# VivianDLi/CryoVIT

Measured on NVIDIA B200. Metric: DINOv2 ViT-g/14 feature slices/sec, higher is better.
Workload: dtype fp16 (norm1 out, attention out, qkv/proj weights) + bf16 (q/k/v, probabilities, norm2 out, w12, FFN hidden, w3) operands, fp32 accumulate

## Files before the change

### cryovit_b200/csrc/attention_tcgen05.cu

```cuda
#include "ptx.cuh"
#include "tmap.h"

namespace cvit {

constexpr int FA_BQ = 128, FA_BK = 128, FA_D = 64;
constexpr int FA_THREADS = 512;
constexpr int FA_REGS_SOFTMAX = 184, FA_REGS_EPILOGUE = 72, FA_REGS_CONTROL = 72;
constexpr int FA_STAGES = 4;
constexpr int FA_TILE_BYTES = 128 * 128;
constexpr int FA_SMEM = (4 + 2 * FA_STAGES) * FA_TILE_BYTES + 4096  + 512  + 1024;
constexpr int FA_TMEM_COLS = 512;
constexpr uint32_t FA_COL_S = 0, FA_COL_P = 256, FA_COL_O = 384;

#ifdef CVIT_FA_TRACE
__device__ __forceinline__ unsigned long long fa_globaltimer() {
  unsigned long long t;
  asm volatile("mov.u64 %0, %%globaltimer;" : "=l"(t));
  return t;
}
#define FA_PROF_DECL uint32_t prof_acc[8] = {0, 0, 0, 0, 0, 0, 0, 0}; const unsigned long long prof_t0 = fa_globaltimer(); uint32_t prof_last = clock()
#define FA_PROF(slot) do { const uint32_t now_ = clock(); prof_acc[slot] += now_ - prof_last; prof_last = now_; } while (0)
#define FA_PROF_DUMP(tiles) do { if (args.trace && blockIdx.x < 4 && lane == 0) {                      \
    long long* d_ = args.trace + (blockIdx.x * 16 + warp) * 10;                                        \
    for (int i_ = 0; i_ < 8; ++i_) d_[i_] = prof_acc[i_];                                              \
    d_[8] = (tiles); d_[9] = (long long)(fa_globaltimer() - prof_t0); } } while (0)
#else
#define FA_PROF_DECL do { } while (0)
#define FA_PROF(slot) do { } while (0)
#define FA_PROF_DUMP(tiles) do { } while (0)
#endif
struct FaArgs {
  long long* trace;
  __nv_bfloat16* out;
  int T, heads, C, slices;
  float scale_log2e;
};

__device__ __forceinline__ uint64_t pack_f32x2(float lo, float hi) {
  uint64_t r;
  asm("mov.b64 %0, {%1, %2};" : "=l"(r) : "f"(lo), "f"(hi));
  return r;
}
__device__ __forceinline__ void unpack_f32x2(uint64_t v, float& lo, float& hi) {
  asm("mov.b64 {%0, %1}, %2;" : "=f"(lo), "=f"(hi) : "l"(v));
}
__device__ __forceinline__ uint64_t fma_f32x2(uint64_t a, uint64_t b, uint64_t c) {
  uint64_t r;
  asm("fma.rn.f32x2 %0, %1, %2, %3;" : "=l"(r) : "l"(a), "l"(b), "l"(c));
  return r;
}
__device__ __forceinline__ uint64_t add_f32x2(uint64_t a, uint64_t b) {
  uint64_t r;
  asm("add.rn.f32x2 %0, %1, %2;" : "=l"(r) : "l"(a), "l"(b));
  return r;
}
__device__ __forceinline__ float fmax3(float a, float b, float c) {
  float r;
  asm("max.f32 %0, %1, %2, %3;" : "=f"(r) : "f"(a), "f"(b), "f"(c));
  return r;
}

template <bool F16, bool OUT16, bool OUT32 = false>
__global__ void __launch_bounds__(FA_THREADS, 1)
attention_tcgen05_kernel(const __grid_constant__ CUtensorMap tmQKV, const FaArgs args) {
  extern __shared__ uint8_t smem_raw[];
  const uint32_t smem_base = (smem_u32(smem_raw) + 1023u) & ~1023u;
  const uint32_t sQ = smem_base;
  const uint32_t sK = smem_base + 4 * FA_TILE_BYTES;
  const uint32_t sV = smem_base + (4 + FA_STAGES) * FA_TILE_BYTES;
  const uint32_t sL = smem_base + (4 + 2 * FA_STAGES) * FA_TILE_BYTES;
  const uint32_t sBar = sL + 4096;
  const uint32_t bar_q = sBar, bar_q_empty = sBar + 16;
  const uint32_t bar_kv_full = sBar + 32;
  const uint32_t bar_kv_empty = sBar + 32 + 8 * FA_STAGES;
  const uint32_t bar_grp = sBar + 32 + 16 * FA_STAGES;
  constexpr uint32_t B_S = 0, B_SFREE = 8, B_P = 16, B_PV = 24, B_OFULL = 32, B_OEMPTY = 40, B_LFULL = 48;
  const uint32_t tmem_slot = bar_grp + 128;
  uint8_t* smem_gen = smem_raw + (smem_base - smem_u32(smem_raw));

  const int warp = threadIdx.x >> 5, lane = threadIdx.x & 31;
  const int T = args.T;
  const int n_tiles = (T + FA_BK - 1) / FA_BK;
  const int n_qt = (T + FA_BQ - 1) / FA_BQ;
  const int n_pairs = (n_qt + 1) >> 1;
  const int total_items = n_pairs * args.heads * args.slices;
  const bool ragged = (T % FA_BK) != 0;
  auto kv_tile = [&](int j) { return ragged ? (j == 0 ? n_tiles - 1 : j - 1) : j; };
  enum { PAIRED = 0, SPLIT = 1, SOLO = 2 };
  auto pair_kind = [&](int pair) { return 2 * pair + 1 < n_qt ? PAIRED : n_tiles > 1 ? SPLIT : SOLO; };
  auto item_kind = [&](int item) { return pair_kind(item % n_pairs); };
  auto mine = [&](int kind, int g, int j) { return kind == PAIRED || (kind == SPLIT ? (j & 1) == g : g == 0); };

  constexpr float FA_RESCALE_LOG2 = F16 ? 8.0f : 16.0f;
  if (threadIdx.x == 0) {
    tma_prefetch_desc(&tmQKV);
    for (int b = 0; b < 2; ++b) {
      mbar_init(bar_q + 8 * b, 1);
      mbar_init(bar_q_empty + 8 * b, 2);
    }
    for (int s = 0; s < FA_STAGES; ++s) {
      mbar_init(bar_kv_full + 8 * s, 1);
      mbar_init(bar_kv_empty + 8 * s, 2);
    }
    for (int g = 0; g < 2; ++g) {
      mbar_init(bar_grp + 64 * g + B_S, 1);
      mbar_init(bar_grp + 64 * g + B_SFREE, 4);
      mbar_init(bar_grp + 64 * g + B_P, 4);
      mbar_init(bar_grp + 64 * g + B_PV, 1);
      mbar_init(bar_grp + 64 * g + B_OFULL, 1);
      mbar_init(bar_grp + 64 * g + B_OEMPTY, 4);
      mbar_init(bar_grp + 64 * g + B_LFULL, 4);
    }
    fence_mbar_init();
  }
  if (warp == 13) tmem_alloc<FA_TMEM_COLS>(tmem_slot);
  tcgen05_fence_before();
  __syncthreads();
  tcgen05_fence_after();
  const uint32_t tmem_base = *reinterpret_cast<volatile uint32_t*>(smem_gen + (tmem_slot - smem_base));

  if (warp >= 12) {
    asm volatile("setmaxnreg.dec.sync.aligned.u32 %0;" ::"n"(FA_REGS_CONTROL));
    if (warp == 12) {
      if (lane == 0) {
        uint32_t kv_it = 0, k = 0;
        for (int item = blockIdx.x; item < total_items; item += gridDim.x, ++k) {
          const int pair = item % n_pairs, bh = item / n_pairs;
          const int head = bh % args.heads, slice = bh / args.heads;
          const int cq = head * FA_D, ck = args.C + head * FA_D, cv = 2 * args.C + head * FA_D;
          const uint32_t qb_ = k & 1, sQk = sQ + qb_ * 2 * FA_TILE_BYTES, bq = bar_q + 8 * qb_;
          mbar_wait(bar_q_empty + 8 * qb_, ((k >> 1) & 1) ^ 1u);
          mbar_arrive_expect_tx(bq, 2 * FA_TILE_BYTES);
          tma_load_3d(sQk, &tmQKV, bq, cq, (2 * pair) * FA_BQ, slice);
          const int qb = item_kind(item) == PAIRED ? 2 * pair + 1 : 2 * pair;
          tma_load_3d(sQk + FA_TILE_BYTES, &tmQKV, bq, cq, qb * FA_BQ, slice);
          for (int j = 0; j < n_tiles; ++j, ++kv_it) {
            const uint32_t s = kv_it % FA_STAGES;
            mbar_wait(bar_kv_empty + 8 * s, ((kv_it / FA_STAGES) & 1) ^ 1u);
            mbar_arrive_expect_tx(bar_kv_full + 8 * s, 2 * FA_TILE_BYTES);
            tma_load_3d(sK + s * FA_TILE_BYTES, &tmQKV, bar_kv_full + 8 * s, ck, kv_tile(j) * FA_BK, slice);
            tma_load_3d(sV + s * FA_TILE_BYTES, &tmQKV, bar_kv_full + 8 * s, cv, kv_tile(j) * FA_BK, slice);
          }
        }
      }
    } else if (warp <= 14) {
      const int g = warp - 13;
      const uint32_t bg = bar_grp + 64 * g;
      constexpr uint32_t idesc_pv = (F16 ? umma_idesc_f16_f32(FA_BQ, FA_D) : umma_idesc_bf16_f32(FA_BQ, FA_D)) | (1u << 16);
      auto n_mma_of = [&](int j) {
        const int valid = min(FA_BK, T - kv_tile(j) * FA_BK);
        return (valid + 15) & ~15;
      };
      FA_PROF_DECL;
      auto issue_s = [&](uint32_t tg, int j, uint32_t k, int commits_q) {
        const uint32_t kv = k * n_tiles + j;
        FA_PROF(7);
        if (tg > 0) mbar_wait(bg + B_SFREE, (tg - 1) & 1);
        FA_PROF(0);
        const uint32_t s = kv % FA_STAGES;
        mbar_wait(bar_kv_full + 8 * s, (kv / FA_STAGES) & 1);
        tcgen05_fence_after();
        FA_PROF(1);
        if (elect_one_sync()) {
          const uint32_t idesc_s = F16 ? umma_idesc_f16_f32(FA_BQ, n_mma_of(j)) : umma_idesc_bf16_f32(FA_BQ, n_mma_of(j));
          const uint64_t qd = umma_smem_desc_kmajor<128>(sQ + ((k & 1) * 2 + g) * FA_TILE_BYTES);
          const uint64_t kd = umma_smem_desc_kmajor<128>(sK + s * FA_TILE_BYTES);
          const uint32_t tS = tmem_base + FA_COL_S + g * 128;
#pragma unroll
          for (int kk = 0; kk < FA_D / 16; ++kk) umma_bf16(tS, qd + 2 * kk, kd + 2 * kk, idesc_s, kk > 0);
          for (int i = 0; i < commits_q; ++i) umma_commit(bar_q_empty + 8 * (k & 1));
          umma_commit(bg + B_S);
        }
        __syncwarp();
        FA_PROF(2);
      };
      auto issue_pv = [&](uint32_t tg, int j, uint32_t kv, bool first, bool last, uint32_t kg, int commits_kv) {
        FA_PROF(7);
        mbar_wait(bg + B_P, tg & 1);
        FA_PROF(3);
        if (first) mbar_wait(bg + B_OEMPTY, (kg & 1) ^ 1u);
        tcgen05_fence_after();
        FA_PROF(4);
        const uint32_t s = kv % FA_STAGES;
        if (elect_one_sync()) {
          const uint32_t tP = tmem_base + FA_COL_P + g * 64, tO = tmem_base + FA_COL_O + g * 64;
          const uint64_t vd = umma_smem_desc_mnmajor_sw128(sV + s * FA_TILE_BYTES, FA_TILE_BYTES);
          if (n_mma_of(j) == FA_BK) {
#pragma unroll
            for (int kk = 0; kk < FA_BK / 16; ++kk)
              umma_bf16_ts(tO, tP + 8 * kk, vd + 128 * kk, idesc_pv, !first || kk != 0);
          } else {
            for (int kk = 0; kk < n_mma_of(j) / 16; ++kk)
              umma_bf16_ts(tO, tP + 8 * kk, vd + 128 * kk, idesc_pv, !first || kk != 0);
          }
          for (int i = 0; i < commits_kv; ++i) umma_commit(bar_kv_empty + 8 * s);
          umma_commit(bg + B_PV);
          if (last) umma_commit(bg + B_OFULL);
        }
        __syncwarp();
        FA_PROF(5);
      };
      struct Cur { int item; uint32_t k; int pair; int kind; int j; };
      const int pair_step = gridDim.x % n_pairs;
      auto cur_valid = [&](const Cur& c) { return c.item < total_items; };
      auto first_j = [&](int kind) { return kind == SPLIT ? g : 0; };
      auto last_j = [&](int kind) { return kind == SPLIT ? n_tiles - 1 - ((n_tiles - 1 - g) & 1) : n_tiles - 1; };
      auto advance = [&](Cur& c) {
        for (;;) {
          ++c.j;
          if (c.j >= n_tiles) {
            c.item += gridDim.x;
            ++c.k;
            c.j = 0;
            if (c.item >= total_items) return;
            c.pair += pair_step;
            if (c.pair >= n_pairs) c.pair -= n_pairs;
            c.kind = pair_kind(c.pair);
          }
          if (mine(c.kind, g, c.j)) return;
        }
      };
      Cur cs{(int)blockIdx.x, 0u, (int)(blockIdx.x % n_pairs), 0, -1}, cp = cs;
      if (cur_valid(cs)) {
        cs.kind = cp.kind = pair_kind(cs.pair);
        advance(cs);
        advance(cp);
      }
      uint32_t ok = 0, obs_q = ~0u;
      int oj = 0;
      auto observe_up_to = [&](const Cur& c) {
        while (ok < c.k || (ok == c.k && oj < c.j)) {
          if (oj == 0) { mbar_wait(bar_q + 8 * (ok & 1), (ok >> 1) & 1); obs_q = ok; }
          const uint32_t kv = ok * n_tiles + oj;
          mbar_wait(bar_kv_full + 8 * (kv % FA_STAGES), (kv / FA_STAGES) & 1);
          if (++oj == n_tiles) { oj = 0; ++ok; }
        }
        if (oj == 0) { mbar_wait(bar_q + 8 * (ok & 1), (ok >> 1) & 1); obs_q = ok; }
        if (++oj == n_tiles) { oj = 0; ++ok; }
      };
      uint32_t ts = 0, tp = 0, kg = 0;
      auto do_s = [&]() {
        FA_PROF(7);
        observe_up_to(cs);
        FA_PROF(6);
        const bool last = cs.j == last_j(cs.kind);
        issue_s(ts, cs.j, cs.k, last ? (cs.kind == SOLO ? 2 : 1) : 0);
        ++ts;
        advance(cs);
      };
      if (cur_valid(cs)) do_s();
      while (cur_valid(cp)) {
        bool s_first = false;
        if (cur_valid(cs)) {
          if (cs.k == obs_q) s_first = true;
          else if (cs.k == obs_q + 1) s_first = __all_sync(0xffffffffu, mbar_try_wait(bar_q + 8 * (cs.k & 1), (cs.k >> 1) & 1));
        }
        if (s_first) do_s();
        const bool first = cp.j == first_j(cp.kind), last = cp.j == last_j(cp.kind);
        issue_pv(tp, cp.j, cp.k * n_tiles + cp.j, first, last, kg, cp.kind == PAIRED ? 1 : 2);
        ++tp;
        if (last) ++kg;
        advance(cp);
        if (!s_first && cur_valid(cs)) do_s();
      }
      FA_PROF(7);
      FA_PROF_DUMP(tp);
    }
  } else if (warp >= 8) {
    asm volatile("setmaxnreg.dec.sync.aligned.u32 %0;" ::"n"(FA_REGS_EPILOGUE));
    const int q = warp & 3;
    const int row = q * 32 + lane;
    const uint32_t t_row = tmem_base + (static_cast<uint32_t>(q * 32) << 16);
    const float* sL_gen = reinterpret_cast<const float*>(smem_gen + (sL - smem_base));
    const float c = args.scale_log2e;
    uint32_t kg[2] = {0, 0};
    for (int item = blockIdx.x; item < total_items; item += gridDim.x) {
      const int pair = item % n_pairs, bh = item / n_pairs, kind = item_kind(item);
      __nv_bfloat16* out_bh = args.out + ((size_t)(bh / args.heads) * T) * args.C + (bh % args.heads) * FA_D;
      float* outf_bh = reinterpret_cast<float*>(args.out) + ((size_t)(bh / args.heads) * T) * args.C + (bh % args.heads) * FA_D;
      if (kind == SPLIT) {
        const int qt = 2 * pair;
        const uint32_t pa = kg[0] & 1, pb = kg[1] & 1;
        ++kg[0];
        ++kg[1];
        mbar_wait(bar_grp + B_LFULL, pa);
        mbar_wait(bar_grp + 64 + B_LFULL, pb);
        const float la = sL_gen[(pa * 2 + 0) * 256 + row], ma = sL_gen[(pa * 2 + 0) * 256 + 128 + row];
        const float lb = sL_gen[(pb * 2 + 1) * 256 + row], mb = sL_gen[(pb * 2 + 1) * 256 + 128 + row];
        const float mm = fmaxf(ma, mb);
        float wa = ex2_approx((ma - mm) * c), wb = ex2_approx((mb - mm) * c);
        const float inv = 1.0f / (wa * la + wb * lb);
        wa *= inv;
        wb *= inv;
        mbar_wait(bar_grp + B_OFULL, pa);
        mbar_wait(bar_grp + 64 + B_OFULL, pb);
        tcgen05_fence_after();
        const bool warp_active = qt * FA_BQ + q * 32 < T;
        if (OUT32 && warp_active) {
          const int tok = qt * FA_BQ + row;
          uint4* dst = reinterpret_cast<uint4*>(outf_bh + (size_t)tok * args.C);
#pragma unroll 1
          for (int hh = 0; hh < 4; ++hh) {
            uint32_t oa[16], o2[16];
            tmem_ld_32x16(t_row + FA_COL_O + hh * 16, oa);
            tmem_ld_32x16(t_row + FA_COL_O + 64 + hh * 16, o2);
            tmem_ld_wait();
#pragma unroll
            for (int i = 0; i < 16; ++i)
              oa[i] = __float_as_uint(round_tf32(__uint_as_float(oa[i]) * wa + __uint_as_float(o2[i]) * wb));
            if (tok < T) {
#pragma unroll
              for (int i = 0; i < 4; ++i) dst[4 * hh + i] = make_uint4(oa[4 * i], oa[4 * i + 1], oa[4 * i + 2], oa[4 * i + 3]);
            }
          }
        } else if (warp_active) {
          const int tok = qt * FA_BQ + row;
          uint4* dst = reinterpret_cast<uint4*>(out_bh + (size_t)tok * args.C);
#pragma unroll 1
          for (int hh = 0; hh < 4; ++hh) {
            uint32_t oa[16], o2[16], ob[8];
            tmem_ld_32x16(t_row + FA_COL_O + hh * 16, oa);
            tmem_ld_32x16(t_row + FA_COL_O + 64 + hh * 16, o2);
            tmem_ld_wait();
#pragma unroll
            for (int i = 0; i < 8; ++i)
              ob[i] = pack_16x2<OUT16>(__uint_as_float(oa[2 * i]) * wa + __uint_as_float(o2[2 * i]) * wb,
                                  __uint_as_float(oa[2 * i + 1]) * wa + __uint_as_float(o2[2 * i + 1]) * wb);
            if (tok < T) {
              dst[2 * hh] = make_uint4(ob[0], ob[1], ob[2], ob[3]);
              dst[2 * hh + 1] = make_uint4(ob[4], ob[5], ob[6], ob[7]);
            }
          }
        }
        tcgen05_fence_before();
        __syncwarp();
        if (lane == 0) {
          mbar_arrive(bar_grp + B_OEMPTY);
          mbar_arrive(bar_grp + 64 + B_OEMPTY);
        }
        continue;
      }
#pragma unroll
      for (int g = 0; g < 2; ++g) {
        if (kind == SOLO && g == 1) continue;
        const int qt = 2 * pair + g;
        const uint32_t bg = bar_grp + 64 * g;
        const uint32_t par = kg[g] & 1;
        ++kg[g];
        mbar_wait(bg + B_LFULL, par);
        const float l = sL_gen[(par * 2 + g) * 256 + row];
        mbar_wait(bg + B_OFULL, par);
        tcgen05_fence_after();
        const bool warp_active = qt * FA_BQ + q * 32 < T;
        if (OUT32 && warp_active) {
          const float inv = 1.0f / l;
          const int tok = qt * FA_BQ + row;
          uint4* dst = reinterpret_cast<uint4*>(outf_bh + (size_t)tok * args.C);
#pragma unroll 1
          for (int hh = 0; hh < 4; ++hh) {
            uint32_t o[16];
            tmem_ld_32x16(t_row + FA_COL_O + g * 64 + hh * 16, o);
            tmem_ld_wait();
#pragma unroll
            for (int i = 0; i < 16; ++i) o[i] = __float_as_uint(round_tf32(__uint_as_float(o[i]) * inv));
            if (tok < T) {
#pragma unroll
              for (int i = 0; i < 4; ++i) dst[4 * hh + i] = make_uint4(o[4 * i], o[4 * i + 1], o[4 * i + 2], o[4 * i + 3]);
            }
          }
        } else if (warp_active) {
          const float inv = 1.0f / l;
          const int tok = qt * FA_BQ + row;
          uint4* dst = reinterpret_cast<uint4*>(out_bh + (size_t)tok * args.C);
#pragma unroll 1
          for (int hh = 0; hh < 2; ++hh) {
            uint32_t o[32];
            tmem_ld_32x32(t_row + FA_COL_O + g * 64 + hh * 32, o);
            tmem_ld_wait();
#pragma unroll
            for (int i = 0; i < 16; ++i) o[i] = pack_16x2<OUT16>(__uint_as_float(o[2 * i]) * inv, __uint_as_float(o[2 * i + 1]) * inv);
            if (tok < T) {
#pragma unroll
              for (int i = 0; i < 4; ++i) dst[4 * hh + i] = make_uint4(o[4 * i], o[4 * i + 1], o[4 * i + 2], o[4 * i + 3]);
            }
          }
        }
        tcgen05_fence_before();
        __syncwarp();
        if (lane == 0) mbar_arrive(bg + B_OEMPTY);
      }
    }
  } else {
    asm volatile("setmaxnreg.inc.sync.aligned.u32 %0;" ::"n"(FA_REGS_SOFTMAX));
    const int g = warp >> 2;
    const int q = warp & 3;
    const int row = q * 32 + lane;
    const uint32_t t_row = tmem_base + (static_cast<uint32_t>(q * 32) << 16);
    const uint32_t tS = t_row + FA_COL_S + g * 128, tP = t_row + FA_COL_P + g * 64, tO = t_row + FA_COL_O + g * 64;
    const uint32_t bg = bar_grp + 64 * g;
    const float c = args.scale_log2e;
    const uint64_t c2 = pack_f32x2(c, c);
    float* sL_gen = reinterpret_cast<float*>(smem_gen + (sL - smem_base));
    uint32_t tile_it = 0, kg = 0;
    bool pending = false;
    FA_PROF_DECL;
    auto publish = [&]() {
      tmem_st_wait();
      tcgen05_fence_before();
      __syncwarp();
      if (lane == 0) mbar_arrive(bg + B_P);
      pending = false;
    };
    for (int item = blockIdx.x; item < total_items; item += gridDim.x) {
      const int pair = item % n_pairs, kind = item_kind(item);
      if (kind == SOLO && g == 1) continue;
      const int qt = kind == PAIRED ? 2 * pair + g : 2 * pair;
      const bool warp_active = qt * FA_BQ + q * 32 < T;
      float m = 0.f, l = 0.f;
      bool first = true;
      for (int j = 0; j < n_tiles; ++j) {
        if (!mine(kind, g, j)) continue;
        FA_PROF(7);
        mbar_wait(bg + B_S, tile_it & 1);
        tcgen05_fence_after();
        FA_PROF(0);
        const int valid = min(FA_BK, T - kv_tile(j) * FA_BK);
        bool pv_seen = tile_it == 0;
        if (warp_active && valid == FA_BK) {
          uint32_t v[128];
          float mx[4] = {-INFINITY, -INFINITY, -INFINITY, -INFINITY};
          tmem_ld_32x32(tS, *reinterpret_cast<uint32_t(*)[32]>(&v[0]));
          if (pending) publish();
#pragma unroll
          for (int ch = 0; ch < 4; ++ch) {
            tmem_ld_wait();
            if (ch < 3) tmem_ld_32x32(tS + (ch + 1) * 32, *reinterpret_cast<uint32_t(*)[32]>(&v[32 * (ch + 1)]));
#pragma unroll
            for (int i = 32 * ch; i < 32 * ch + 32; i += 8) {
#pragma unroll
              for (int u = 0; u < 4; ++u)
                mx[u] = fmax3(mx[u], __uint_as_float(v[i + 2 * u]), __uint_as_float(v[i + 2 * u + 1]));
            }
          }
          tcgen05_fence_before();
          __syncwarp();
          if (lane == 0) mbar_arrive(bg + B_SFREE);
          FA_PROF(1);
          const float mt = fmaxf(fmaxf(mx[0], mx[1]), fmaxf(mx[2], mx[3]));
          if (first) {
            m = mt;
          } else {
            const bool need = (mt - m) * c > FA_RESCALE_LOG2;
            if (__any_sync(0xffffffffu, need)) {
              mbar_wait(bg + B_PV, (tile_it - 1) & 1);
              tcgen05_fence_after();
              pv_seen = true;
              const float f = need ? ex2_approx((m - mt) * c) : 1.0f;
#pragma unroll 1
              for (int hh = 0; hh < 4; ++hh) {
                uint32_t o[16];
                tmem_ld_32x16(tO + hh * 16, o);
                tmem_ld_wait();
#pragma unroll
                for (int i = 0; i < 16; ++i) o[i] = __float_as_uint(__uint_as_float(o[i]) * f);
                tmem_st_32x16(tO + hh * 16, o);
              }
              l *= f;
              if (need) m = mt;
            }
          }
          FA_PROF(2);
          const float nmc = -m * c;
          const uint64_t nmc2 = pack_f32x2(nmc, nmc);
          uint64_t ls[4] = {0ull, 0ull, 0ull, 0ull};
#pragma unroll
          for (int i = 0; i < 64; ++i) {
            const uint64_t t2 = fma_f32x2(pack_f32x2(__uint_as_float(v[2 * i]), __uint_as_float(v[2 * i + 1])), c2, nmc2);
            float t0, t1;
            unpack_f32x2(t2, t0, t1);
            const float p0 = ex2_approx(t0), p1 = ex2_approx(t1);
            ls[i & 3] = add_f32x2(ls[i & 3], pack_f32x2(p0, p1));
            v[i] = pack_16x2<F16>(p0, p1);
          }
          {
            float a0, a1;
            unpack_f32x2(add_f32x2(add_f32x2(ls[0], ls[1]), add_f32x2(ls[2], ls[3])), a0, a1);
            l += a0 + a1;
          }
          FA_PROF(4);
          if (!pv_seen) {
            mbar_wait(bg + B_PV, (tile_it - 1) & 1);
            tcgen05_fence_after();
          }
#pragma unroll
          for (int ch = 0; ch < 4; ++ch)
            tmem_st_32x16(tP + ch * 16, *reinterpret_cast<uint32_t(*)[16]>(&v[16 * ch]));
          pending = true;
          if (j + 1 == n_tiles || (kind == SPLIT && j + 2 >= n_tiles)) publish();
// ... 10 lines not shown
#pragma unroll
          for (int i = 0; i < 16; ++i)
            if (i < valid) mt = fmaxf(mt, __uint_as_float(v[i]));
          m = mt;
          const float nmc = -m * c;
          uint32_t pk[8];
#pragma unroll
          for (int i = 0; i < 8; ++i) {
            const float p0 = 2 * i < valid ? ex2_approx(fmaf(__uint_as_float(v[2 * i]), c, nmc)) : 0.f;
            const float p1 = 2 * i + 1 < valid ? ex2_approx(fmaf(__uint_as_float(v[2 * i + 1]), c, nmc)) : 0.f;
            l += p0 + p1;
            pk[i] = pack_16x2<F16>(p0, p1);
          }
          if (!pv_seen) {
            mbar_wait(bg + B_PV, (tile_it - 1) & 1);
            tcgen05_fence_after();
          }
          tmem_st_32x8(tP, pk);
          pending = true;
          if (j + 1 == n_tiles || (kind == SPLIT && j + 2 >= n_tiles)) publish();
          FA_PROF(6);
        } else {
          if (pending) publish();
          if (!pv_seen) {
            mbar_wait(bg + B_PV, (tile_it - 1) & 1);
            tcgen05_fence_after();
          }
          if (warp_active) {
            const int nch = (valid + 15) >> 4;
            float mt = -INFINITY;
            for (int ch = 0; ch < nch; ++ch) {
              uint32_t v[16];
              tmem_ld_32x16(tS + ch * 16, v);
              tmem_ld_wait();
#pragma unroll
              for (int i = 0; i < 16; ++i)
                if (ch * 16 + i < valid) mt = fmaxf(mt, __uint_as_float(v[i]));
            }
            if (first) {
              m = mt;
            } else {
              const bool need = (mt - m) * c > FA_RESCALE_LOG2;
              if (__any_sync(0xffffffffu, need)) {
                const float f = need ? ex2_approx((m - mt) * c) : 1.0f;
#pragma unroll 1
                for (int hh = 0; hh < 2; ++hh) {
                  uint32_t o[32];
                  tmem_ld_32x32(tO + hh * 32, o);
                  tmem_ld_wait();
#pragma unroll
                  for (int i = 0; i < 32; ++i) o[i] = __float_as_uint(__uint_as_float(o[i]) * f);
                  tmem_st_32x32(tO + hh * 32, o);
                }
                l *= f;
                if (need) m = mt;
              }
            }
            const float nmc = -m * c;
            for (int ch = 0; ch < nch; ++ch) {
              uint32_t v[16];
              tmem_ld_32x16(tS + ch * 16, v);
              tmem_ld_wait();
              uint32_t pk[8];
#pragma unroll
              for (int i = 0; i < 8; ++i) {
                const int k0 = ch * 16 + 2 * i;
                const float p0 = k0 < valid ? ex2_approx(fmaf(__uint_as_float(v[2 * i]), c, nmc)) : 0.f;
                const float p1 = k0 + 1 < valid ? ex2_approx(fmaf(__uint_as_float(v[2 * i + 1]), c, nmc)) : 0.f;
                l += p0 + p1;
                pk[i] = pack_16x2<F16>(p0, p1);
              }
              tmem_st_32x8(tP + ch * 8, pk);
            }
          }
          tcgen05_fence_before();
          __syncwarp();
          if (lane == 0) mbar_arrive(bg + B_SFREE);
          publish();
          FA_PROF(6);
        }
        first = false;
        ++tile_it;
      }
      sL_gen[((kg & 1) * 2 + g) * 256 + row] = l;
      sL_gen[((kg & 1) * 2 + g) * 256 + 128 + row] = m;
      ++kg;
      __syncwarp();
      if (lane == 0) mbar_arrive(bg + B_LFULL);
    }
    FA_PROF(7);
    FA_PROF_DUMP(tile_it);
  }

  tcgen05_fence_before();
  __syncthreads();
  if (warp == 13) {
    __syncwarp();
    tcgen05_fence_after();
    tmem_dealloc<FA_TMEM_COLS>(tmem_base);
  }
}

}

using namespace cvit;

#ifdef CVIT_FA_TRACE
static long long* g_fa_trace = nullptr;
extern "C" void cvit_fa_set_trace(long long* p) { g_fa_trace = p; }
#endif

template <bool F16, bool OUT16, bool OUT32 = false>
static int attention_fwd(const void* qkv, void* out, int64_t n_slices, int64_t tokens, int64_t heads, int64_t head_dim,
                         void* stream) {
  if (!qkv || !out || n_slices <= 0 || tokens <= 0 || heads <= 0) {
    set_error("attention: bad arguments");
    return CVIT_ERR_INVALID;
  }
  if (head_dim != FA_D) {
    set_error("attention: head_dim=%lld unsupported (64 only: every DINOv2 variant)", (long long)head_dim);
    return CVIT_ERR_UNSUPPORTED;
  }
  if (((tokens + FA_BQ - 1) / FA_BQ) * heads * n_slices > 0x7fffffffll) {
    set_error("attention: too many work items");
    return CVIT_ERR_UNSUPPORTED;
  }
  const int64_t C = heads * FA_D;
  CUtensorMap tm;
  uint64_t dims[3] = {(uint64_t)(3 * C), (uint64_t)tokens, (uint64_t)n_slices};
  uint64_t strides[3] = {0, (uint64_t)(3 * C) * 2, (uint64_t)tokens * 3 * C * 2};
  uint32_t box[3] = {FA_D, FA_BK, 1};
  int rc = encode_tmap(&tm, F16 ? TmapDtype::F16 : TmapDtype::BF16, 3, qkv, dims, strides, box, 128);
  if (rc) return rc;
  static bool configured = false;
  if (!configured) {
    cudaError_t e = cudaFuncSetAttribute(attention_tcgen05_kernel<F16, OUT16, OUT32>, cudaFuncAttributeMaxDynamicSharedMemorySize, FA_SMEM);
    if (e != cudaSuccess) {
      set_error("attention: cudaFuncSetAttribute: %s", cudaGetErrorString(e));
      return CVIT_ERR_CUDA;
    }
    configured = true;
  }
  FaArgs a;
#ifdef CVIT_FA_TRACE
  a.trace = g_fa_trace;
#else
  a.trace = nullptr;
#endif
  a.out = static_cast<__nv_bfloat16*>(out);
  a.T = (int)tokens;
  a.heads = (int)heads;
  a.C = (int)C;
  a.slices = (int)n_slices;
  a.scale_log2e = 0.125f * 1.4426950408889634f;
  const int n_qt = (int)((tokens + FA_BQ - 1) / FA_BQ);
  const int64_t items = (int64_t)((n_qt + 1) / 2) * heads * n_slices;
  int grid = num_sms();
  if (grid > items) grid = (int)items;
  attention_tcgen05_kernel<F16, OUT16, OUT32><<<grid, FA_THREADS, FA_SMEM, (cudaStream_t)stream>>>(tm, a);
  return check_launch("attention_tcgen05_kernel");
}

extern "C" int cvit_attention_fwd_bf16(const void* qkv, void* out, int64_t n_slices, int64_t tokens, int64_t heads,
                                       int64_t head_dim, void* stream) {
  return attention_fwd<false, false>(qkv, out, n_slices, tokens, heads, head_dim, stream);
}

extern "C" int cvit_attention_fwd_f16(const void* qkv, void* out, int64_t n_slices, int64_t tokens, int64_t heads,
                                      int64_t head_dim, void* stream) {
  return attention_fwd<true, true>(qkv, out, n_slices, tokens, heads, head_dim, stream);
}

extern "C" int cvit_attention_fwd_fmt(const void* qkv, void* out, int64_t n_slices, int64_t tokens, int64_t heads,
                                      int64_t head_dim, int fmt, void* stream) {
// ... 11 lines not shown
```

### cryovit_b200/csrc/ptx.cuh

```cuda
#pragma once
#include <cuda.h>
#include <cuda_bf16.h>
#include <cuda_fp16.h>
#include <cuda_runtime.h>
#include <stdint.h>
#include <stdio.h>

namespace cvit {

__device__ __forceinline__ uint32_t smem_u32(const void* p) {
  return static_cast<uint32_t>(__cvta_generic_to_shared(p));
}

__device__ __forceinline__ void mbar_init(uint32_t bar, uint32_t count) {
  asm volatile("mbarrier.init.shared::cta.b64 [%0], %1;" ::"r"(bar), "r"(count) : "memory");
}
__device__ __forceinline__ void fence_mbar_init() {
  asm volatile("fence.mbarrier_init.release.cluster;" ::: "memory");
}
__device__ __forceinline__ void fence_proxy_async_smem() {
  asm volatile("fence.proxy.async.shared::cta;" ::: "memory");
}
__device__ __forceinline__ void mbar_arrive(uint32_t bar) {
  asm volatile("mbarrier.arrive.shared::cta.b64 _, [%0];" ::"r"(bar) : "memory");
// ... 178 lines not shown

__device__ __forceinline__ uint32_t cluster_ctarank() {
  uint32_t r;
  asm volatile("mov.u32 %0, %%cluster_ctarank;" : "=r"(r));
  return r;
}
__device__ __forceinline__ void cluster_sync_all() {
  asm volatile("barrier.cluster.arrive.release.aligned;\nbarrier.cluster.wait.acquire.aligned;" ::: "memory");
}
__device__ __forceinline__ uint32_t mapa_cluster(uint32_t addr, uint32_t rank) {
  uint32_t r;
  asm volatile("mapa.shared::cluster.u32 %0, %1, %2;" : "=r"(r) : "r"(addr), "r"(rank));
  return r;
}
__device__ __forceinline__ void mbar_arrive_cluster(uint32_t cluster_bar) {
  asm volatile("mbarrier.arrive.release.cluster.shared::cluster.b64 _, [%0];" ::"r"(cluster_bar) : "memory");
}
__device__ __forceinline__ void tma_load_2d_pair(uint32_t dst, const CUtensorMap* m, uint32_t cluster_bar, int c0, int c1) {
  asm volatile(
      "cp.async.bulk.tensor.2d.cta_group::2.shared::cluster.global.mbarrier::complete_tx::bytes [%0], [%1, {%3, "
      "%4}], [%2];" ::"r"(dst),
      "l"(m), "r"(cluster_bar), "r"(c0), "r"(c1)
      : "memory");
}
__device__ __forceinline__ void tma_load_4d_pair(uint32_t dst, const CUtensorMap* m, uint32_t cluster_bar, int c0, int c1,
                                                 int c2, int c3) {
  asm volatile(
      "cp.async.bulk.tensor.4d.cta_group::2.shared::cluster.global.mbarrier::complete_tx::bytes [%0], [%1, {%3, %4, "
      "%5, %6}], [%2];" ::"r"(dst),
      "l"(m), "r"(cluster_bar), "r"(c0), "r"(c1), "r"(c2), "r"(c3)
      : "memory");
}
template <int NCOLS>
__device__ __forceinline__ void tmem_alloc_pair(uint32_t dst_smem) {
  asm volatile("tcgen05.alloc.cta_group::2.sync.aligned.shared::cta.b32 [%0], %1;" ::"r"(dst_smem), "n"(NCOLS) : "memory");
  asm volatile("tcgen05.relinquish_alloc_permit.cta_group::2.sync.aligned;" ::: "memory");
}
template <int NCOLS>
__device__ __forceinline__ void tmem_dealloc_pair(uint32_t taddr) {
  asm volatile("tcgen05.dealloc.cta_group::2.sync.aligned.b32 %0, %1;" ::"r"(taddr), "n"(NCOLS) : "memory");
}
__device__ __forceinline__ void umma_bf16_pair(uint32_t d_tmem, uint64_t adesc, uint64_t bdesc, uint32_t idesc,
                                               uint32_t accumulate) {
  asm volatile(
      "{\n"
      ".reg .pred p;\n"
      "setp.ne.b32 p, %4, 0;\n"
      "tcgen05.mma.cta_group::2.kind::f16 [%0], %1, %2, %3, p;\n"
      "}\n" ::"r"(d_tmem),
      "l"(adesc), "l"(bdesc), "r"(idesc), "r"(accumulate)
      : "memory");
}
__device__ __forceinline__ void umma_tf32_pair(uint32_t d_tmem, uint64_t adesc, uint64_t bdesc, uint32_t idesc,
                                               uint32_t accumulate) {
  asm volatile(
      "{\n"
      ".reg .pred p;\n"
      "setp.ne.b32 p, %4, 0;\n"
      "tcgen05.mma.cta_group::2.kind::tf32 [%0], %1, %2, %3, p;\n"
      "}\n" ::"r"(d_tmem),
      "l"(adesc), "l"(bdesc), "r"(idesc), "r"(accumulate)
      : "memory");
}
__device__ __forceinline__ void umma_commit_pair(uint32_t bar) {
  asm volatile(
      "{\n"
      ".reg .b16 m;\n"
      "mov.b16 m, 3;\n"
      "tcgen05.commit.cta_group::2.mbarrier::arrive::one.shared::cluster.multicast::cluster.b64 [%0], m;\n"
      "}\n" ::"r"(bar)
      : "memory");
}

template <int SWIZZLE_BYTES>
__device__ __forceinline__ uint64_t umma_smem_desc_kmajor(uint32_t smem_addr) {
  constexpr uint64_t layout = SWIZZLE_BYTES == 128 ? 2ull : SWIZZLE_BYTES == 64 ? 4ull : 6ull;
  constexpr uint64_t sbo = (8ull * SWIZZLE_BYTES) >> 4;
  return static_cast<uint64_t>((smem_addr & 0x3ffffu) >> 4) | (1ull << 16) | (sbo << 32) | (1ull << 46) |
         (layout << 61);
}
__device__ __forceinline__ uint64_t umma_smem_desc_mnmajor_sw128(uint32_t smem_addr, uint32_t lbo_bytes) {
  return static_cast<uint64_t>((smem_addr & 0x3ffffu) >> 4) | (static_cast<uint64_t>((lbo_bytes >> 4) & 0x3fff) << 16) |
         (static_cast<uint64_t>(1024 >> 4) << 32) | (1ull << 46) | (2ull << 61);
}
__host__ __device__ constexpr uint32_t umma_idesc_bf16_f32(int M, int N) {
  return (1u << 4) | (1u << 7) | (1u << 10) | (static_cast<uint32_t>(N >> 3) << 17) |
         (static_cast<uint32_t>(M >> 4) << 24);
}
__host__ __device__ constexpr uint32_t umma_idesc_f16_f32(int M, int N) {
  return (1u << 4) | (static_cast<uint32_t>(N >> 3) << 17) | (static_cast<uint32_t>(M >> 4) << 24);
}
constexpr uint32_t UMMA_IDESC_BF16_BITS = (1u << 7) | (1u << 10);
__host__ __device__ constexpr uint32_t umma_idesc_tf32_f32(int M, int N) {
  return (1u << 4) | (2u << 7) | (2u << 10) | (static_cast<uint32_t>(N >> 3) << 17) |
         (static_cast<uint32_t>(M >> 4) << 24);
}
__device__ __forceinline__ void umma_tf32(uint32_t d_tmem, uint64_t adesc, uint64_t bdesc, uint32_t idesc,
                                          uint32_t accumulate) {
  asm volatile(
      "{\n"
      ".reg .pred p;\n"
      "setp.ne.b32 p, %4, 0;\n"
      "tcgen05.mma.cta_group::1.kind::tf32 [%0], %1, %2, %3, p;\n"
      "}\n" ::"r"(d_tmem),
      "l"(adesc), "l"(bdesc), "r"(idesc), "r"(accumulate)
      : "memory");
}

__device__ __forceinline__ float gelu_erf_exact(float x) { return 0.5f * x * (1.0f + erff(x * 0.70710678118654752f)); }
__device__ __forceinline__ float ex2_approx(float x) {
  float y;
  asm("ex2.approx.ftz.f32 %0, %1;" : "=f"(y) : "f"(x));
  return y;
}
__device__ __forceinline__ float rcp_approx(float x) {
  float y;
  asm("rcp.approx.ftz.f32 %0, %1;" : "=f"(y) : "f"(x));
  return y;
}
__device__ __forceinline__ float gelu_erf_as(float x) {
  const float z = fabsf(x) * 0.70710678118654752f;
  const float t = rcp_approx(fmaf(0.3275911f, z, 1.0f));
  float p = fmaf(1.061405429f, t, -1.453152027f);
  p = fmaf(p, t, 1.421413741f);
  p = fmaf(p, t, -0.284496736f);
  p = fmaf(p, t, 0.254829592f);
  p *= t;
  const float e = ex2_approx(z * z * -1.4426950408889634f);
  const float erf_abs = fmaf(-p, e, 1.0f);
  const float h = 0.5f * x;
  return fmaf(h, copysignf(erf_abs, x), h);
}
__device__ __forceinline__ float gelu_erf(float x) {
  constexpr float L2E = 1.4426950408889634f;
  const float x2 = fminf(x * x, 36.0f);
  float q = fmaf(7.030335764e-4f * L2E, x2, -7.401129204e-2f * L2E);
  q = fmaf(q, x2, -1.5950157686f * L2E);
  const float e = ex2_approx(q * x);
  return x * rcp_approx(1.0f + e);
}
__device__ __forceinline__ void gelu_erf2(float& a, float& b) {
  constexpr float L2E = 1.4426950408889634f;
  uint64_t x, x2, q, t;
  asm("mov.b64 %0, {%1, %2};" : "=l"(x) : "f"(a), "f"(b));
  asm("mul.rn.f32x2 %0, %1, %1;" : "=l"(x2) : "l"(x));
  float x2a, x2b;
  asm("mov.b64 {%0, %1}, %2;" : "=f"(x2a), "=f"(x2b) : "l"(x2));
  x2a = fminf(x2a, 36.0f);
  x2b = fminf(x2b, 36.0f);
  asm("mov.b64 %0, {%1, %2};" : "=l"(x2) : "f"(x2a), "f"(x2b));
  uint64_t c2, c1, c0, one;
  asm("mov.b64 %0, {%1, %1};" : "=l"(c2) : "f"(7.030335764e-4f * L2E));
  asm("mov.b64 %0, {%1, %1};" : "=l"(c1) : "f"(-7.401129204e-2f * L2E));
  asm("mov.b64 %0, {%1, %1};" : "=l"(c0) : "f"(-1.5950157686f * L2E));
  asm("mov.b64 %0, {%1, %1};" : "=l"(one) : "f"(1.0f));
  asm("fma.rn.f32x2 %0, %1, %2, %3;" : "=l"(q) : "l"(c2), "l"(x2), "l"(c1));
  asm("fma.rn.f32x2 %0, %1, %2, %3;" : "=l"(q) : "l"(q), "l"(x2), "l"(c0));
  asm("mul.rn.f32x2 %0, %1, %2;" : "=l"(t) : "l"(q), "l"(x));
  float ta, tb;
  asm("mov.b64 {%0, %1}, %2;" : "=f"(ta), "=f"(tb) : "l"(t));
  uint64_t e;
  asm("mov.b64 %0, {%1, %2};" : "=l"(e) : "f"(ex2_approx(ta)), "f"(ex2_approx(tb)));
  asm("add.rn.f32x2 %0, %1, %2;" : "=l"(e) : "l"(e), "l"(one));
  float da, db;
  asm("mov.b64 {%0, %1}, %2;" : "=f"(da), "=f"(db) : "l"(e));
  uint64_t r;
  asm("mov.b64 %0, {%1, %2};" : "=l"(r) : "f"(rcp_approx(da)), "f"(rcp_approx(db)));
  asm("mul.rn.f32x2 %0, %1, %2;" : "=l"(r) : "l"(x), "l"(r));
  asm("mov.b64 {%0, %1}, %2;" : "=f"(a), "=f"(b) : "l"(r));
}
__device__ __forceinline__ float gelu_grad(float z) {
  const float u = fabsf(z) * 0.70710678118654752f;
  const float t = rcp_approx(fmaf(0.3275911f, u, 1.0f));
  float p = fmaf(1.061405429f, t, -1.453152027f);
  p = fmaf(p, t, 1.421413741f);
  p = fmaf(p, t, -0.284496736f);
  p = fmaf(p, t, 0.254829592f);
  p *= t;
  const float e = ex2_approx(u * u * -1.4426950408889634f);
  const float cdf = fmaf(0.5f, copysignf(fmaf(-p, e, 1.0f), z), 0.5f);
  return fmaf(z * 0.3989422804014327f, e, cdf);
}

enum { ACT_NONE = 0, ACT_GELU = 1, ACT_DUAL = 2, ACT_GELU_GRAD = 3 };
__device__ __forceinline__ uint32_t act_gelu_grad_pair(float a, float b, uint32_t z2) {
  const float z0 = __uint_as_float(z2 << 16), z1 = __uint_as_float(z2 & 0xffff0000u);
  uint32_t r;
  asm("cvt.rn.bf16x2.f32 %0, %1, %2;" : "=r"(r) : "f"(b * gelu_grad(z1)), "f"(a * gelu_grad(z0)));
  return r;
}
__device__ __forceinline__ float silu(float x) { return __fdividef(x, 1.0f + ex2_approx(-1.4426950408889634f * x)); }
__device__ __forceinline__ uint32_t pack_bf16x2(float lo, float hi) {
  __nv_bfloat162 v = __floats2bfloat162_rn(lo, hi);
  return *reinterpret_cast<uint32_t*>(&v);
}
__device__ __forceinline__ uint32_t pack_f16x2(float lo, float hi) {
  __half2 v = __floats2half2_rn(lo, hi);
  return *reinterpret_cast<uint32_t*>(&v);
}
__device__ __forceinline__ float round_tf32(float x) {
  uint32_t r;
  asm("cvt.rna.tf32.f32 %0, %1;" : "=r"(r) : "f"(x));
  return __uint_as_float(r & 0xffffe000u);
}
template <bool F16>
__device__ __forceinline__ uint32_t pack_16x2(float lo, float hi) {
  return F16 ? pack_f16x2(lo, hi) : pack_bf16x2(lo, hi);
}
__device__ __forceinline__ void st_global_v8(void* p, const uint32_t (&v)[8]) {
  asm volatile("st.global.v8.b32 [%0], {%1, %2, %3, %4, %5, %6, %7, %8};" ::"l"(p), "r"(v[0]), "r"(v[1]), "r"(v[2]), "r"(v[3]),
               "r"(v[4]), "r"(v[5]), "r"(v[6]), "r"(v[7])
               : "memory");
}
__device__ __forceinline__ float warp_sum(float v) {
#pragma unroll
  for (int o = 16; o > 0; o >>= 1) v += __shfl_xor_sync(0xffffffffu, v, o);
  return v;
}
__device__ __forceinline__ float warp_max(float v) {
#pragma unroll
  for (int o = 16; o > 0; o >>= 1) v = fmaxf(v, __shfl_xor_sync(0xffffffffu, v, o));
  return v;
}

}
```

Measured before the change: 409.1.

## Add transposed narrow-N tail path for nearly-empty final query tile

Adds a TAIL item kind for the final query tile when it holds at most 16 rows. In that case S is computed transposed (keys as M=128, queries as N=16) and P is staged in swizzled shared memory, so PV runs as a narrow V^T·P MMA instead of a full 128-row tile. The softmax warps reduce the per-query max and sum across warps through named barriers and a shared scratch area, and the epilogue merges the two groups' partial results. This avoids spending full-tile MMA and softmax work on a mostly padded tile. In exchange it adds a complex extra code path, more synchronisation and extra shared memory.

```diff
diff --git a/cryovit_b200/csrc/attention_tcgen05.cu b/cryovit_b200/csrc/attention_tcgen05.cu
--- a/cryovit_b200/csrc/attention_tcgen05.cu
+++ b/cryovit_b200/csrc/attention_tcgen05.cu
@@ -8,7 +8,10 @@
 constexpr int FA_REGS_SOFTMAX = 184, FA_REGS_EPILOGUE = 72, FA_REGS_CONTROL = 72;
 constexpr int FA_STAGES = 4;
 constexpr int FA_TILE_BYTES = 128 * 128;
-constexpr int FA_SMEM = (4 + 2 * FA_STAGES) * FA_TILE_BYTES + 4096  + 512  + 1024;
+constexpr int FA_TAIL_N = 16;
+constexpr int FA_PT_BYTES = FA_BK * FA_TAIL_N * 2;
+constexpr int FA_SMEM = (4 + 2 * FA_STAGES) * FA_TILE_BYTES + 2 * FA_PT_BYTES + 4096  +
+                        1024  + 512  + 1024;
 constexpr int FA_TMEM_COLS = 512;
 constexpr uint32_t FA_COL_S = 0, FA_COL_P = 256, FA_COL_O = 384;
 
@@ -20,14 +23,14 @@
 }
 #define FA_PROF_DECL uint32_t prof_acc[8] = {0, 0, 0, 0, 0, 0, 0, 0}; const unsigned long long prof_t0 = fa_globaltimer(); uint32_t prof_last = clock()
 #define FA_PROF(slot) do { const uint32_t now_ = clock(); prof_acc[slot] += now_ - prof_last; prof_last = now_; } while (0)
-#define FA_PROF_DUMP(tiles) do { if (args.trace && blockIdx.x < 4 && lane == 0) {                      \
-    long long* d_ = args.trace + (blockIdx.x * 16 + warp) * 10;                                        \
+#define FA_PROF_DUMP(tiles, tail_tiles) do { if (args.trace && blockIdx.x < 4 && lane == 0) {          \
+    long long* d_ = args.trace + (blockIdx.x * 16 + warp) * 12;                                        \
     for (int i_ = 0; i_ < 8; ++i_) d_[i_] = prof_acc[i_];                                              \
-    d_[8] = (tiles); d_[9] = (long long)(fa_globaltimer() - prof_t0); } } while (0)
+    d_[8] = (tiles); d_[9] = (long long)(fa_globaltimer() - prof_t0); d_[10] = (tail_tiles); d_[11] = 0; } } while (0)
 #else
 #define FA_PROF_DECL do { } while (0)
 #define FA_PROF(slot) do { } while (0)
-#define FA_PROF_DUMP(tiles) do { } while (0)
+#define FA_PROF_DUMP(tiles, tail_tiles) do { } while (0)
 #endif
 struct FaArgs {
   long long* trace;
@@ -68,8 +71,10 @@
   const uint32_t sQ = smem_base;
   const uint32_t sK = smem_base + 4 * FA_TILE_BYTES;
   const uint32_t sV = smem_base + (4 + FA_STAGES) * FA_TILE_BYTES;
-  const uint32_t sL = smem_base + (4 + 2 * FA_STAGES) * FA_TILE_BYTES;
-  const uint32_t sBar = sL + 4096;
+  const uint32_t sPt = smem_base + (4 + 2 * FA_STAGES) * FA_TILE_BYTES;
+  const uint32_t sL = sPt + 2 * FA_PT_BYTES;
+  const uint32_t sRed = sL + 4096;
+  const uint32_t sBar = sRed + 1024;
   const uint32_t bar_q = sBar, bar_q_empty = sBar + 16;
   const uint32_t bar_kv_full = sBar + 32;
   const uint32_t bar_kv_empty = sBar + 32 + 8 * FA_STAGES;
@@ -86,10 +91,14 @@
   const int total_items = n_pairs * args.heads * args.slices;
   const bool ragged = (T % FA_BK) != 0;
   auto kv_tile = [&](int j) { return ragged ? (j == 0 ? n_tiles - 1 : j - 1) : j; };
-  enum { PAIRED = 0, SPLIT = 1, SOLO = 2 };
-  auto pair_kind = [&](int pair) { return 2 * pair + 1 < n_qt ? PAIRED : n_tiles > 1 ? SPLIT : SOLO; };
+  enum { PAIRED = 0, SPLIT = 1, SOLO = 2, TAIL = 3 };
+  const int tail_r = T - (n_qt - 1) * FA_BQ;
+  auto pair_kind = [&](int pair) {
+    return 2 * pair + 1 < n_qt ? PAIRED : n_tiles == 1 ? SOLO : tail_r <= FA_TAIL_N ? TAIL : SPLIT;
+  };
   auto item_kind = [&](int item) { return pair_kind(item % n_pairs); };
-  auto mine = [&](int kind, int g, int j) { return kind == PAIRED || (kind == SPLIT ? (j & 1) == g : g == 0); };
+  auto split_sched = [](int kind) { return kind == SPLIT || kind == TAIL; };
+  auto mine = [&](int kind, int g, int j) { return kind == PAIRED || (split_sched(kind) ? (j & 1) == g : g == 0); };
 
   constexpr float FA_RESCALE_LOG2 = F16 ? 8.0f : 16.0f;
   if (threadIdx.x == 0) {
@@ -147,12 +156,15 @@
       const int g = warp - 13;
       const uint32_t bg = bar_grp + 64 * g;
       constexpr uint32_t idesc_pv = (F16 ? umma_idesc_f16_f32(FA_BQ, FA_D) : umma_idesc_bf16_f32(FA_BQ, FA_D)) | (1u << 16);
+      constexpr uint32_t idesc_st = F16 ? umma_idesc_f16_f32(FA_BK, FA_TAIL_N) : umma_idesc_bf16_f32(FA_BK, FA_TAIL_N);
+      constexpr uint32_t idesc_ot =
+          (F16 ? umma_idesc_f16_f32(FA_D, FA_TAIL_N) : umma_idesc_bf16_f32(FA_D, FA_TAIL_N)) | (1u << 15) | (1u << 16);
       auto n_mma_of = [&](int j) {
         const int valid = min(FA_BK, T - kv_tile(j) * FA_BK);
         return (valid + 15) & ~15;
       };
       FA_PROF_DECL;
-      auto issue_s = [&](uint32_t tg, int j, uint32_t k, int commits_q) {
+      auto issue_s = [&](uint32_t tg, int j, uint32_t k, int commits_q, bool tail) {
         const uint32_t kv = k * n_tiles + j;
         FA_PROF(7);
         if (tg > 0) mbar_wait(bg + B_SFREE, (tg - 1) & 1);
@@ -166,15 +178,20 @@
           const uint64_t qd = umma_smem_desc_kmajor<128>(sQ + ((k & 1) * 2 + g) * FA_TILE_BYTES);
           const uint64_t kd = umma_smem_desc_kmajor<128>(sK + s * FA_TILE_BYTES);
           const uint32_t tS = tmem_base + FA_COL_S + g * 128;
-#pragma unroll
-          for (int kk = 0; kk < FA_D / 16; ++kk) umma_bf16(tS, qd + 2 * kk, kd + 2 * kk, idesc_s, kk > 0);
+          if (tail) {
+#pragma unroll
+            for (int kk = 0; kk < FA_D / 16; ++kk) umma_bf16(tS, kd + 2 * kk, qd + 2 * kk, idesc_st, kk > 0);
+          } else {
+#pragma unroll
+            for (int kk = 0; kk < FA_D / 16; ++kk) umma_bf16(tS, qd + 2 * kk, kd + 2 * kk, idesc_s, kk > 0);
+          }
           for (int i = 0; i < commits_q; ++i) umma_commit(bar_q_empty + 8 * (k & 1));
           umma_commit(bg + B_S);
         }
         __syncwarp();
         FA_PROF(2);
       };
-      auto issue_pv = [&](uint32_t tg, int j, uint32_t kv, bool first, bool last, uint32_t kg, int commits_kv) {
+      auto issue_pv = [&](uint32_t tg, int j, uint32_t kv, bool first, bool last, uint32_t kg, int commits_kv, bool tail) {
         FA_PROF(7);
         mbar_wait(bg + B_P, tg & 1);
         FA_PROF(3);
@@ -185,7 +202,11 @@
         if (elect_one_sync()) {
           const uint32_t tP = tmem_base + FA_COL_P + g * 64, tO = tmem_base + FA_COL_O + g * 64;
           const uint64_t vd = umma_smem_desc_mnmajor_sw128(sV + s * FA_TILE_BYTES, FA_TILE_BYTES);
-          if (n_mma_of(j) == FA_BK) {
+          if (tail) {
+            const uint64_t pd = umma_smem_desc_mnmajor_sw32(sPt + g * FA_PT_BYTES, FA_PT_BYTES);
+            for (int kk = 0; kk < n_mma_of(j) / 16; ++kk)
+              umma_bf16(tO, vd + 128 * kk, pd + 32 * kk, idesc_ot, !first || kk != 0);
+          } else if (n_mma_of(j) == FA_BK) {
 #pragma unroll
             for (int kk = 0; kk < FA_BK / 16; ++kk)
               umma_bf16_ts(tO, tP + 8 * kk, vd + 128 * kk, idesc_pv, !first || kk != 0);
@@ -203,8 +224,8 @@
       struct Cur { int item; uint32_t k; int pair; int kind; int j; };
       const int pair_step = gridDim.x % n_pairs;
       auto cur_valid = [&](const Cur& c) { return c.item < total_items; };
-      auto first_j = [&](int kind) { return kind == SPLIT ? g : 0; };
-      auto last_j = [&](int kind) { return kind == SPLIT ? n_tiles - 1 - ((n_tiles - 1 - g) & 1) : n_tiles - 1; };
+      auto first_j = [&](int kind) { return split_sched(kind) ? g : 0; };
+      auto last_j = [&](int kind) { return split_sched(kind) ? n_tiles - 1 - ((n_tiles - 1 - g) & 1) : n_tiles - 1; };
       auto advance = [&](Cur& c) {
         for (;;) {
           ++c.j;
@@ -244,7 +265,7 @@
         observe_up_to(cs);
         FA_PROF(6);
         const bool last = cs.j == last_j(cs.kind);
-        issue_s(ts, cs.j, cs.k, last ? (cs.kind == SOLO ? 2 : 1) : 0);
+        issue_s(ts, cs.j, cs.k, last ? (cs.kind == SOLO ? 2 : 1) : 0, cs.kind == TAIL);
         ++ts;
         advance(cs);
       };
@@ -257,14 +278,14 @@
         }
         if (s_first) do_s();
         const bool first = cp.j == first_j(cp.kind), last = cp.j == last_j(cp.kind);
-        issue_pv(tp, cp.j, cp.k * n_tiles + cp.j, first, last, kg, cp.kind == PAIRED ? 1 : 2);
+        issue_pv(tp, cp.j, cp.k * n_tiles + cp.j, first, last, kg, cp.kind == PAIRED ? 1 : 2, cp.kind == TAIL);
         ++tp;
         if (last) ++kg;
         advance(cp);
         if (!s_first && cur_valid(cs)) do_s();
       }
       FA_PROF(7);
-      FA_PROF_DUMP(tp);
+      FA_PROF_DUMP(tp, 0);
     }
   } else if (warp >= 8) {
     asm volatile("setmaxnreg.dec.sync.aligned.u32 %0;" ::"n"(FA_REGS_EPILOGUE));
@@ -278,6 +299,48 @@
       const int pair = item % n_pairs, bh = item / n_pairs, kind = item_kind(item);
       __nv_bfloat16* out_bh = args.out + ((size_t)(bh / args.heads) * T) * args.C + (bh % args.heads) * FA_D;
       float* outf_bh = reinterpret_cast<float*>(args.out) + ((size_t)(bh / args.heads) * T) * args.C + (bh % args.heads) * FA_D;
+      if (kind == TAIL) {
+        const int tok0 = 2 * pair * FA_BQ;
+        const uint32_t pa = kg[0] & 1, pb = kg[1] & 1;
+        ++kg[0];
+        ++kg[1];
+        mbar_wait(bar_grp + B_LFULL, pa);
+        mbar_wait(bar_grp + 64 + B_LFULL, pb);
+        mbar_wait(bar_grp + B_OFULL, pa);
+        mbar_wait(bar_grp + 64 + B_OFULL, pb);
+        tcgen05_fence_after();
+        uint32_t oa[FA_TAIL_N], o2[FA_TAIL_N];
+        tmem_ld_32x16(t_row + FA_COL_O, oa);
+        tmem_ld_32x16(t_row + FA_COL_O + 64, o2);
+        tmem_ld_wait();
+        const float* La = sL_gen + (pa * 2 + 0) * 256;
+        const float* Lb = sL_gen + (pb * 2 + 1) * 256;
+        const int d = q * 16 + lane;
+#pragma unroll
+        for (int i = 0; i < FA_TAIL_N; ++i) {
+          if (i >= tail_r) break;
+          const float la = (La[i] + La[16 + i]) + (La[32 + i] + La[48 + i]), ma = La[128 + i];
+          const float lb = (Lb[i] + Lb[16 + i]) + (Lb[32 + i] + Lb[48 + i]), mb = Lb[128 + i];
+          const float mm = fmaxf(ma, mb);
+          float wa = ex2_approx((ma - mm) * c), wb = ex2_approx((mb - mm) * c);
+          const float inv = 1.0f / (wa * la + wb * lb);
+          wa *= inv;
+          wb *= inv;
+          const float o = __uint_as_float(oa[i]) * wa + __uint_as_float(o2[i]) * wb;
+          if (lane < 16) {
+            const size_t at = (size_t)(tok0 + i) * args.C + d;
+            if (OUT32) outf_bh[at] = round_tf32(o);
+            else reinterpret_cast<uint16_t*>(out_bh)[at] = static_cast<uint16_t>(pack_16x2<OUT16>(o, 0.f) & 0xffffu);
+          }
+        }
+        tcgen05_fence_before();
+        __syncwarp();
+        if (lane == 0) {
+          mbar_arrive(bar_grp + B_OEMPTY);
+          mbar_arrive(bar_grp + 64 + B_OEMPTY);
+        }
+        continue;
+      }
       if (kind == SPLIT) {
         const int qt = 2 * pair;
         const uint32_t pa = kg[0] & 1, pb = kg[1] & 1;
@@ -411,9 +474,117 @@
       if (lane == 0) mbar_arrive(bg + B_P);
       pending = false;
     };
+    auto sums_slot_free = [&]() {
+      if (kg > 0) mbar_wait(bg + B_OEMPTY, (kg - 1) & 1);
+    };
+    uint32_t tail_tiles = 0;
     for (int item = blockIdx.x; item < total_items; item += gridDim.x) {
       const int pair = item % n_pairs, kind = item_kind(item);
       if (kind == SOLO && g == 1) continue;
+      if (kind == TAIL) {
+        float tm[FA_TAIL_N], tl[FA_TAIL_N];
+#pragma unroll
+        for (int i = 0; i < FA_TAIL_N; ++i) tm[i] = tl[i] = 0.f;
+        float* red = reinterpret_cast<float*>(smem_gen + (sRed - smem_base)) + g * 128;
+        const uint32_t pt_row = sPt + g * FA_PT_BYTES + row * 32, pt_sw = ((row >> 2) & 1) << 4;
+        for (int j = g; j < n_tiles; j += 2) {
+          FA_PROF(7);
+          mbar_wait(bg + B_S, tile_it & 1);
+          tcgen05_fence_after();
+          FA_PROF(0);
+          uint32_t v[FA_TAIL_N];
+          tmem_ld_32x16(tS, v);
+          if (pending) publish();
+          tmem_ld_wait();
+          tcgen05_fence_before();
+          __syncwarp();
+          if (lane == 0) mbar_arrive(bg + B_SFREE);
+          const bool key_ok = kv_tile(j) * FA_BK + row < T;
+          float* rp = red + (tile_it & 1) * 64;
+          float wmax = -INFINITY;
+#pragma unroll
+          for (int i = 0; i < FA_TAIL_N; ++i) {
+            if (i >= tail_r) break;
+            const float x = warp_max(key_ok ? __uint_as_float(v[i]) : -INFINITY);
+            if (lane == i) wmax = x;
+          }
+          if (lane < FA_TAIL_N) rp[q * FA_TAIL_N + lane] = wmax;
+          named_bar_sync(1 + g, 128);
+          bool pv_seen = tile_it == 0;
+          float f[FA_TAIL_N];
+          bool rescale = false;
+#pragma unroll
+          for (int i = 0; i < FA_TAIL_N; ++i) {
+            f[i] = 1.0f;
+            if (i >= tail_r) continue;
+            const float mt = fmaxf(fmaxf(rp[i], rp[16 + i]), fmaxf(rp[32 + i], rp[48 + i]));
+            if (j == g) {
+              tm[i] = mt;
+            } else if ((mt - tm[i]) * c > FA_RESCALE_LOG2) {
+              f[i] = ex2_approx((tm[i] - mt) * c);
+              tm[i] = mt;
+              rescale = true;
+            }
+          }
+          if (rescale) {
+            mbar_wait(bg + B_PV, (tile_it - 1) & 1);
+            tcgen05_fence_after();
+            pv_seen = true;
+            uint32_t o[FA_TAIL_N];
+            tmem_ld_32x16(tO, o);
+            tmem_ld_wait();
+#pragma unroll
+            for (int i = 0; i < FA_TAIL_N; ++i) {
+              o[i] = __float_as_uint(__uint_as_float(o[i]) * f[i]);
+              tl[i] *= f[i];
+            }
+            tmem_st_32x16(tO, o);
+          }
+          uint32_t pk[FA_TAIL_N / 2];
+#pragma unroll
+          for (int i = 0; i < FA_TAIL_N / 2; ++i) {
+            float p[2];
+#pragma unroll
+            for (int h = 0; h < 2; ++h) {
+              const int qi = 2 * i + h;
+              p[h] = key_ok && qi < tail_r ? ex2_approx(fmaf(__uint_as_float(v[qi]), c, -tm[qi] * c)) : 0.f;
+              tl[qi] += p[h];
+            }
+            pk[i] = pack_16x2<F16>(p[0], p[1]);
+          }
+          if (!pv_seen) {
+            mbar_wait(bg + B_PV, (tile_it - 1) & 1);
+            tcgen05_fence_after();
+          }
+          st_shared_v4(pt_row + pt_sw, pk[0], pk[1], pk[2], pk[3]);
+          st_shared_v4(pt_row + (pt_sw ^ 16u), pk[4], pk[5], pk[6], pk[7]);
+          fence_proxy_async_smem();
+          publish();
+          FA_PROF(3);
+          ++tile_it;
+          ++tail_tiles;
+        }
+        float ls = 0.f, ms = 0.f;
+#pragma unroll
+        for (int i = 0; i < FA_TAIL_N; ++i) {
+          if (i >= tail_r) break;
+          const float s = warp_sum(tl[i]);
+          if (lane == i) {
+            ls = s;
+            ms = tm[i];
+          }
+        }
+        sums_slot_free();
+        float* dst = sL_gen + ((kg & 1) * 2 + g) * 256;
+        if (lane < FA_TAIL_N) {
+          dst[q * FA_TAIL_N + lane] = ls;
+          dst[128 + lane] = ms;
+        }
+        ++kg;
+        __syncwarp();
+        if (lane == 0) mbar_arrive(bg + B_LFULL);
+        continue;
+      }
       const int qt = kind == PAIRED ? 2 * pair + g : 2 * pair;
       const bool warp_active = qt * FA_BQ + q * 32 < T;
       float m = 0.f, l = 0.f;
@@ -590,6 +761,7 @@
         first = false;
         ++tile_it;
       }
+      sums_slot_free();
       sL_gen[((kg & 1) * 2 + g) * 256 + row] = l;
       sL_gen[((kg & 1) * 2 + g) * 256 + 128 + row] = m;
       ++kg;
@@ -597,7 +769,7 @@
       if (lane == 0) mbar_arrive(bg + B_LFULL);
     }
     FA_PROF(7);
-    FA_PROF_DUMP(tile_it);
+    FA_PROF_DUMP(tile_it, tail_tiles);
   }
 
   tcgen05_fence_before();
diff --git a/cryovit_b200/csrc/ptx.cuh b/cryovit_b200/csrc/ptx.cuh
--- a/cryovit_b200/csrc/ptx.cuh
+++ b/cryovit_b200/csrc/ptx.cuh
@@ -284,6 +284,10 @@
 __device__ __forceinline__ uint64_t umma_smem_desc_mnmajor_sw128(uint32_t smem_addr, uint32_t lbo_bytes) {
   return static_cast<uint64_t>((smem_addr & 0x3ffffu) >> 4) | (static_cast<uint64_t>((lbo_bytes >> 4) & 0x3fff) << 16) |
          (static_cast<uint64_t>(1024 >> 4) << 32) | (1ull << 46) | (2ull << 61);
+}
+__device__ __forceinline__ uint64_t umma_smem_desc_mnmajor_sw32(uint32_t smem_addr, uint32_t lbo_bytes) {
+  return static_cast<uint64_t>((smem_addr & 0x3ffffu) >> 4) | (static_cast<uint64_t>((lbo_bytes >> 4) & 0x3fff) << 16) |
+         (static_cast<uint64_t>(256 >> 4) << 32) | (1ull << 46) | (6ull << 61);
 }
 __host__ __device__ constexpr uint32_t umma_idesc_bf16_f32(int M, int N) {
   return (1u << 4) | (1u << 7) | (1u << 10) | (static_cast<uint32_t>(N >> 3) << 17) |
@@ -414,6 +418,12 @@
                "r"(v[4]), "r"(v[5]), "r"(v[6]), "r"(v[7])
                : "memory");
 }
+__device__ __forceinline__ void named_bar_sync(uint32_t id, uint32_t nthreads) {
+  asm volatile("bar.sync %0, %1;" ::"r"(id), "r"(nthreads) : "memory");
+}
+__device__ __forceinline__ void st_shared_v4(uint32_t addr, uint32_t a, uint32_t b, uint32_t c, uint32_t d) {
+  asm volatile("st.shared.v4.b32 [%0], {%1, %2, %3, %4};" ::"r"(addr), "r"(a), "r"(b), "r"(c), "r"(d) : "memory");
+}
 __device__ __forceinline__ float warp_sum(float v) {
 #pragma unroll
   for (int o = 16; o > 0; o >>= 1) v += __shfl_xor_sync(0xffffffffu, v, o);
```

Result: slower. 403.6, median of 6 (-1.3%).
